# ittiam-systems/libxaac

Hardware: AMD Instinct MI355X
Metric: decoded audio frames/s (1024-spl IMDCT + complex QMF + HQ SBR + parametric stereo, HE-AACv2) (higher is better)
Workload: dtype int32

## Files before the change

libxaac_amd/csrc/sbr_ps_frame.h:

```cpp
#ifndef XAAC_SBR_PS_FRAME_H
#define XAAC_SBR_PS_FRAME_H

#include <stddef.h>

#include "sbr_ps.h"

#ifndef XP_T
#define XP_T(i)
#endif

#define XP_NO_PS_SCALE 0x7fffffff
#define XP_MAX_SEG (XAAC_PS_MAX_ENV + 2)

#if defined(__HIPCC__)
#define XP_UNROLL _Pragma("unroll")
#define XP_NOUNROLL _Pragma("nounroll")
#define XP_LAMBDA_INLINE __attribute__((always_inline))
#else
#define XP_UNROLL
#define XP_NOUNROLL
#define XP_LAMBDA_INLINE
#endif

struct XpFrameWork {
  union {
    int32_t hyb_u[3][2][44];
    int32_t gsum[8][56];
    int32_t peak[32][20];
    uint32_t dl[32][13];
  };
  int32_t hyb_l[32][20];
  union {
    int32_t binpw[32][20];
    int16_t ratio[32][20];
  };
  uint32_t ap_h[32][11];
  uint32_t seg_hd[XP_MAX_SEG][4][24];
};
template <bool B>
struct XpBool {
  static constexpr bool value = B;
};

FX_HD int xp_popc(uint32_t v) { return __builtin_popcount(v); }
FX_HD int xp_clz(uint32_t v) { return __builtin_clz(v); }
FX_HD uint32_t xp_pack16(int16_t lo, int16_t hi) { return (uint32_t)(uint16_t)lo | ((uint32_t)(uint16_t)hi << 16); }
FX_HD int16_t xp_lo16(uint32_t v) { return (int16_t)(v & 0xffffu); }
FX_HD int16_t xp_hi16(uint32_t v) { return (int16_t)(v >> 16); }

FX_HD int32_t xp_dot2(uint32_t a, uint32_t b) {
#if defined(__HIP_DEVICE_COMPILE__)
  int32_t r;
  asm("v_dot2_i32_i16 %0, %1, %2, 0" : "=v"(r) : "v"(a), "v"(b));
  return r;
#else
  return (int32_t)((uint32_t)((int32_t)xp_lo16(a) * xp_lo16(b)) + (uint32_t)((int32_t)xp_hi16(a) * xp_hi16(b)));
#endif
}
FX_HD int16_t xp_seg_coeff(uint32_t hd, int n) { return (int16_t)(xp_hi16(hd) + n * xp_lo16(hd)); }
FX_HD uint32_t xp_load_pair(const int16_t *p) {
#if defined(__HIP_DEVICE_COMPILE__)
  typedef uint32_t __attribute__((may_alias)) xp_u32_alias;
  return *reinterpret_cast<const xp_u32_alias *>(p);
#else
  return xp_pack16(p[0], p[1]);
#endif
}
struct XpPhase {
  uint32_t re_pair, im_pair;
};
FX_HD XpPhase xp_phase_pairs(int16_t re, int16_t im) {
  XpPhase p;
  p.re_pair = xp_pack16(re, (int16_t)-im);
  p.im_pair = xp_pack16(im, re);
  return p;
}
FX_HD uint32_t xp_q15_pair(int32_t a, int32_t b) {
  return (((uint32_t)a >> 15) & 0xffffu) | (((uint32_t)b << 1) & 0xffff0000u);
}
FX_HD uint32_t xp_hi_pair(int32_t a, int32_t b) {
#if defined(__HIP_DEVICE_COMPILE__)
  return __builtin_amdgcn_perm((uint32_t)b, (uint32_t)a, 0x07060302u);
#else
  return ((uint32_t)a >> 16) | ((uint32_t)b & 0xffff0000u);
#endif
}
FX_HD uint32_t xp_mult16_shl_pair(uint32_t p, int32_t f2) {
#if defined(__HIP_DEVICE_COMPILE__)
  return xp_hi_pair(__mul24(xp_lo16(p), f2), __mul24(xp_hi16(p), f2));
#else
  return xp_hi_pair((int32_t)((uint32_t)(int32_t)xp_lo16(p) * (uint32_t)f2), (int32_t)((uint32_t)(int32_t)xp_hi16(p) * (uint32_t)f2));
#endif
}
FX_HD int32_t xp_m16x16_shl_pre(int16_t a, int32_t b2) {
#if defined(__HIP_DEVICE_COMPILE__)
  return __mul24(a, b2);
#else
  return (int32_t)((uint32_t)(int32_t)a * (uint32_t)b2);
#endif
}
FX_HD uint32_t xp_add16_pair(uint32_t a, uint32_t b) {
#if defined(__HIP_DEVICE_COMPILE__)
  typedef short xp_short2 __attribute__((ext_vector_type(2)));
  return __builtin_bit_cast(uint32_t, (xp_short2)(__builtin_bit_cast(xp_short2, a) + __builtin_bit_cast(xp_short2, b)));
#else
  return ((a + b) & 0xffffu) | ((a & 0xffff0000u) + (b & 0xffff0000u));
#endif
}
FX_HD uint32_t xp_sub16_pair(uint32_t a, uint32_t b) {
#if defined(__HIP_DEVICE_COMPILE__)
  typedef short xp_short2 __attribute__((ext_vector_type(2)));
  return __builtin_bit_cast(uint32_t, (xp_short2)(__builtin_bit_cast(xp_short2, a) - __builtin_bit_cast(xp_short2, b)));
#else
  return ((a - b) & 0xffffu) | ((a & 0xffff0000u) - (b & 0xffff0000u));
#endif
}
FX_HD uint32_t xp_allpass_packed(uint32_t &d0, uint32_t new_pair, const XpPhase &ph, uint32_t &e0, uint32_t &e1, uint32_t &e2,
                                 const XpPhase &p0, const XpPhase &p1, const XpPhase &p2, int16_t decay0, int16_t decay1,
                                 int16_t decay2) {
  uint32_t in = xp_q15_pair(xp_dot2(d0, ph.re_pair), xp_dot2(d0, ph.im_pair));
  d0 = new_pair;
  uint32_t *e[3] = {&e0, &e1, &e2};
  const XpPhase *pp[3] = {&p0, &p1, &p2};
  const int32_t decay2x[3] = {2 * decay0, 2 * decay1, 2 * decay2};
  XP_UNROLL
  for (int m = 0; m < 3; m++) {
    const uint32_t s = *e[m];
    const uint32_t t = xp_sub16_pair(xp_q15_pair(xp_dot2(s, pp[m]->re_pair), xp_dot2(s, pp[m]->im_pair)),
                                     xp_mult16_shl_pair(in, decay2x[m]));
    *e[m] = xp_add16_pair(in, xp_mult16_shl_pair(t, decay2x[m]));
    in = t;
  }
  return in;
}

FX_HD int32_t xp_adj_word(int32_t v, int shift) {
  if (shift > 31) shift = 31;
  if (shift < -31) shift = -31;
  const int shl = shift > 0 ? shift : 0, shr = shift < 0 ? -shift : 0;
  return (int32_t)((uint32_t)v << shl) >> shr;
}

FX_HD int32_t xp_bin_power_hyb(const XpTables *T, int bin, const int32_t *re, const int32_t *im) {
  if (bin < 2) {
    const int a = bin == 0 ? 0 : 4, b = bin == 0 ? 5 : 1;
    int32_t pw = xp_power(re[a], im[a]);
    pw = fx_add_sat(pw, fx_mul32x16(re[b], (int16_t)(re[b] >> 16)));
    return fx_add_sat(pw, fx_mul32x16(im[b], (int16_t)(im[b] >> 16)));
  }
  const int sb = T->borders_group[bin + 2];
  return xp_power(re[sb], im[sb]);
}

template <int NS = 32, class PS>
FX_HD int xp_ps_frame(const XsCx &cx, const XpTables *T, PS *ps, const xaac_ps_frame *pf, XpFrameWork *w, int32_t *xl,
                      int32_t *xr, int lb_scale, int ov_lb_scale, int hb_scale, int st_syn, int lsb, int usb,
                      int ps_scale_done = XP_NO_PS_SCALE) {
  static_assert(NS == 32 || NS == 30, "frames of 32 or 30 QMF slots");
#if defined(__HIP_DEVICE_COMPILE__)
  int32_t p1v[3][2], p3re[32], p3im[32];
  {
    const int l1 = cx.lane & 31;
    XP_UNROLL
    for (int b = 0; b < 3; b++) {
      p1v[b][0] = xl[(l1 + 6) * 128 + b];
      p1v[b][1] = xl[(l1 + 6) * 128 + 64 + b];
    }
    XP_UNROLL
    for (int l = 0; l < 32; l++) {
      p3re[l] = NS == 32 || l < NS ? xl[l * 128 + cx.lane] : 0;
      p3im[l] = NS == 32 || l < NS ? xl[l * 128 + 64 + cx.lane] : 0;
    }
  }
#endif
  const int ps_scale = ps_scale_done != XP_NO_PS_SCALE ? ps_scale_done : xp_init_ps_scale(cx, ps, lb_scale, ov_lb_scale, hb_scale);
  const int ov_lb_shift = ps_scale - ov_lb_scale, lb_shift = ps_scale - lb_scale, hb_shift = ps_scale - hb_scale;
  const int common_shift = (st_syn - ps_scale) - 8;
  XP_T(1);

  XS_PAR(l, 0, NS) {
    const int shiftdelay = l < NS - 6 ? 0 : (int16_t)(lb_scale - ps_scale);
    for (int b = 0; b < 3; b++) {
      const int sha = l + 6 < NS ? (b < lsb ? lb_shift : (b < usb ? hb_shift : 0)) : 0;
      for (int c = 0; c < 2; c++) {
#if defined(__HIP_DEVICE_COMPILE__)
        int32_t v = xp_adj_word(p1v[b][c], sha);
#else
        int32_t v = xp_adj_word(xl[(l + 6) * 128 + 64 * c + b], sha);
#endif
        v = shiftdelay < 0 ? fx_shl(v, -shiftdelay) : fx_shr(v, shiftdelay);
        w->hyb_u[b][c][12 + l] = v;
      }
    }
  }
  XS_PAR(i, 0, 12)
    for (int b = 0; b < 3; b++) {
      w->hyb_u[b][0][i] = ps->hyb_buf[b][0][i];
      w->hyb_u[b][1][i] = ps->hyb_buf[b][1][i];
    }
  cx.sync();
  XS_PAR(l, 0, NS) {
    int32_t re[8], im[8];
    xp_filt_8ch(T, &w->hyb_u[0][0][l], &w->hyb_u[0][1][l], re, im);
    for (int k = 0; k < 6; k++) {
      w->hyb_l[l][k] = re[k];
      w->hyb_l[l][10 + k] = im[k];
    }
  }
  XS_PAR(i, 0, 64) {
    const int b = 1 + (i >> 5), l = i & 31;
    if (NS != 32 && l >= NS) continue;
    int32_t re[2], im[2];
    xp_filt_2ch(T, &w->hyb_u[b][0][l], &w->hyb_u[b][1][l], re, im);
    w->hyb_l[l][4 + 2 * b] = re[0];
    w->hyb_l[l][5 + 2 * b] = re[1];
    w->hyb_l[l][14 + 2 * b] = im[0];
    w->hyb_l[l][15 + 2 * b] = im[1];
  }
  XS_PAR(i, 0, 12)
    for (int b = 0; b < 3; b++) {
      ps->hyb_buf[b][0][i] = w->hyb_u[b][0][NS + i];
      ps->hyb_buf[b][1][i] = w->hyb_u[b][1][NS + i];
    }
  cx.sync();
  XP_T(2);

  XS_PAR(g, 0, XAAC_PS_GROUPS) {
    w->seg_hd[0][0][g] = xp_pack16(ps->delta_h11_h12[2 * g], ps->H11_H12[2 * g]);
    w->seg_hd[0][1][g] = xp_pack16(ps->delta_h11_h12[2 * g + 1], ps->H11_H12[2 * g + 1]);
    w->seg_hd[0][2][g] = xp_pack16(ps->delta_h21_h22[2 * g], ps->H21_H22[2 * g]);
    w->seg_hd[0][3][g] = xp_pack16(ps->delta_h21_h22[2 * g + 1], ps->H21_H22[2 * g + 1]);
  }
  const int usb_prev = cx.uni(ps->usb);
  uint32_t seg_mask = 0;
  int clear_slot = NS;
  {
    int env = 0, nseg = 1;
    int next = cx.uni(pf->border_position[0]);
    for (int l = 0; l < NS; l++) {
      if (l == next) {
        if (env == 0) clear_slot = l;
        cx.sync();
        xp_rot_env_coeffs(cx, T, ps, pf, env);
        XS_PAR(g, 0, XAAC_PS_GROUPS) {
          w->seg_hd[nseg][0][g] = xp_pack16(ps->delta_h11_h12[2 * g], ps->H11_H12[2 * g]);
          w->seg_hd[nseg][1][g] = xp_pack16(ps->delta_h11_h12[2 * g + 1], ps->H11_H12[2 * g + 1]);
          w->seg_hd[nseg][2][g] = xp_pack16(ps->delta_h21_h22[2 * g], ps->H21_H22[2 * g]);
          w->seg_hd[nseg][3][g] = xp_pack16(ps->delta_h21_h22[2 * g + 1], ps->H21_H22[2 * g + 1]);
        }
        seg_mask |= 1u << l;
        nseg++;
        env++;
        next = env <= XAAC_PS_MAX_ENV ? cx.uni(pf->border_position[env]) : 64;
      }
    }
  }
  cx.sync();
  XP_T(3);

  {
    XP_UNROLL
    for (int c = 0; c < 4; c++) {
      XS_PAR(sb, 0, 64) {
        int32_t rre[8], rim[8];
        XP_UNROLL
        for (int ls = 0; ls < 8; ls++) {
#if defined(__HIP_DEVICE_COMPILE__)
          rre[ls] = p3re[8 * c + ls];
          rim[ls] = p3im[8 * c + ls];
#else
          rre[ls] = xl[(8 * c + ls) * 128 + sb];
          rim[ls] = xl[(8 * c + ls) * 128 + 64 + sb];
#endif
        }
        const int gsh = sb < 11 ? 0 : (sb < 18 ? 1 : (sb < 23 ? 2 : (sb < 35 ? 3 : 4)));
        const bool own_bin = sb >= 3 && sb < 9;
        int32_t *dst = sb < 3 ? &w->gsum[0][55] : (own_bin ? &w->binpw[8 * c][sb + 5] : &w->gsum[0][sb - 9]);
        const int dstride = own_bin ? 20 : 56;
        XP_UNROLL
        for (int ls = 0; ls < 8; ls++) {
          const int l = 8 * c + ls;
          const int usb_l = l >= clear_slot ? usb : usb_prev;
          const int sh = sb < lsb ? (l < 6 ? ov_lb_shift : lb_shift) : (sb < usb ? hb_shift : 0);
          const int32_t re = xp_adj_word(rre[ls], sh), im = xp_adj_word(rim[ls], sh);
          const int32_t pw = xp_power(re, im);
          dst[ls * dstride] = own_bin ? pw : (sb < usb_l ? (pw >> gsh) : 0);
        }
      }
      cx.sync();
      XS_PAR(i, 0, 48) {
        const int ls = i / 6, g = i % 6;
        const int b0 = T->borders_group[16 + g], b1 = T->borders_group[17 + g];
        int32_t acc = 0;
#if defined(__HIP_DEVICE_COMPILE__) && !defined(XP_OLD_GSUM)
        for (int sb = b0; sb < b1; sb += 8) {
          int32_t t[8];
          XP_UNROLL
          for (int j = 0; j < 8; j++) t[j] = w->gsum[ls][(sb + j < b1 ? sb + j : b1 - 1) - 9];
          XP_UNROLL
          for (int j = 0; j < 8; j++) acc = fx_add_sat(acc, sb + j < b1 ? t[j] : 0);
        }
#else
        for (int sb = b0; sb < b1; sb++) acc = fx_add_sat(acc, w->gsum[ls][sb - 9]);
#endif
        w->binpw[8 * c + ls][14 + g] = acc;
      }
      cx.sync();
    }
  }
  XS_PAR(i, 0, 8 * NS) {
    const int l = i >> 3, bin = i & 7;
    w->binpw[l][bin] = xp_bin_power_hyb(T, bin, &w->hyb_l[l][0], &w->hyb_l[l][10]);
  }
  cx.sync();
  XP_T(4);

  XS_PAR(bin, 0, 20) {
    int32_t pd = ps->peak_decay_diff[bin], pdp = ps->peak_decay_diff_prev[bin], nrg = ps->energy_prev[bin];
    int32_t pin[NS];
    XP_UNROLL
    for (int l = 0; l < NS; l++) pin[l] = w->binpw[l][bin];
    XP_UNROLL
    for (int l = 0; l < NS; l++) {
      int32_t pw = fx_shl(pin[l], 1);
      if (pw < 0) pw = 0;
      pd = fx_mul32x16_shl(pd, 0x620a);
      if (pw > pd) pd = pw;
      pdp = fx_add_sat(fx_mul32x16_shl(pdp, 0x6000), fx_sub_sat(pd, pw) >> 2);
      nrg = fx_add_sat(fx_mul32x16_shl(nrg, 0x6000), pw >> 2);
      w->binpw[l][bin] = nrg;
      w->peak[l][bin] = fx_add_sat(pdp, pdp >> 1);
    }
    ps->peak_decay_diff[bin] = pd;
    ps->peak_decay_diff_prev[bin] = pdp;
    ps->energy_prev[bin] = nrg;
  }
  cx.sync();
  for (int i0 = 0; i0 < 20 * NS; i0 += 64) {
    int16_t q = 0;
    XS_PAR(i, i0, (20 * NS) % 64 == 0 || i0 + 64 < 20 * NS ? i0 + 64 : 20 * NS) {
      const int32_t pk = (&w->peak[0][0])[i], nrg = (&w->binpw[0][0])[i];
      q = pk <= nrg ? (int16_t)0x7fff : (int16_t)xp_divide16_pos(nrg, pk);
#if !defined(__HIP_DEVICE_COMPILE__)
      (&w->ratio[0][0])[i] = q;
#endif
    }
#if defined(__HIP_DEVICE_COMPILE__)
    cx.sync();
    (&w->ratio[0][0])[i0 + cx.lane] = q;
    cx.sync();
#endif
  }
  cx.sync();
  XP_T(5);

  {
    const int idx0 = cx.uni(ps->idx), idx_long0 = cx.uni(ps->idx_long);
    const int is0 = cx.uni(ps->idx_ser[0]), is1 = cx.uni(ps->idx_ser[1]), is2 = cx.uni(ps->idx_ser[2]);
    const int clear_lo = (usb > usb_prev && usb_prev) ? usb_prev : 64;
    const int clear_hi = usb < 23 ? usb : 23;
    const int p14_0 = idx_long0 % 14;
    const int cs_right = common_shift < 0 ? (-common_shift > 31 ? 31 : -common_shift) : 0;
    uint32_t events = seg_mask | (1u << 6) | (1u << 14);
    if (clear_slot < NS) events |= 1u << clear_slot;
    if (clear_slot + 14 < NS) events |= 1u << (clear_slot + 14);
    XS_PAR(sb, 0, 64) {
      const int qmf_chain = sb >= 3 && sb < 23, hyb_chain = sb >= 32 && sb < 42, chain = qmf_chain || hyb_chain;
      const int csb = qmf_chain ? sb : (hyb_chain ? sb - 32 : 3);
      const int di = 9 + 3 * (csb - 3);
      const int16_t *ph = hyb_chain ? &T->frac_delay_phase_fac_qmf_sub_re_im[2 * csb] : &T->frac_delay_phase_fac_qmf_re_im[2 * csb];
      const int16_t *pser = hyb_chain ? &T->frac_delay_phase_fac_qmf_sub_ser_re_im[2 * csb] : &T->frac_delay_phase_fac_qmf_ser_re_im[2 * csb];
      const int pstep = hyb_chain ? 32 : 64;
      const XpPhase phase = xp_phase_pairs(ph[0], ph[1]);
      const XpPhase ps0 = xp_phase_pairs(pser[0], pser[1]), ps1 = xp_phase_pairs(pser[pstep], pser[pstep + 1]),
                    ps2 = xp_phase_pairs(pser[2 * pstep], pser[2 * pstep + 1]);
      const int16_t dec0 = hyb_chain ? T->rev_link_decay_ser[0] : T->decay_scale_factor[qmf_chain ? di : 9];
      const int16_t dec1 = hyb_chain ? T->rev_link_decay_ser[1] : T->decay_scale_factor[qmf_chain ? di + 1 : 10];
      const int16_t dec2 = hyb_chain ? T->rev_link_decay_ser[2] : T->decay_scale_factor[qmf_chain ? di + 2 : 11];
      uint32_t d0[2] = {0, 0}, r0[3] = {0, 0, 0}, r1[4] = {0, 0, 0, 0}, r2[5] = {0, 0, 0, 0, 0};
      if (chain) {
        XP_UNROLL
        for (int j = 0; j < 2; j++) {
          const int16_t *q = hyb_chain ? &ps->sub[(idx0 + j) % 2][2 * csb] : &ps->ap[(idx0 + j) % 2][2 * csb];
          d0[j] = xp_pack16(q[0], q[1]);
        }
        XP_UNROLL
        for (int j = 0; j < 3; j++) {
          const int16_t *q = hyb_chain ? &ps->sub_ser[(is0 + j) % 3][0][2 * csb] : &ps->ser[(is0 + j) % 3][0][2 * csb];
          r0[j] = xp_pack16(q[0], q[1]);
        }
        XP_UNROLL
        for (int j = 0; j < 4; j++) {
          const int16_t *q = hyb_chain ? &ps->sub_ser[(is1 + j) % 4][1][2 * csb] : &ps->ser[(is1 + j) % 4][1][2 * csb];
          r1[j] = xp_pack16(q[0], q[1]);
        }
        XP_UNROLL
        for (int j = 0; j < 5; j++) {
          const int16_t *q = hyb_chain ? &ps->sub_ser[(is2 + j) % 5][2][2 * csb] : &ps->ser[(is2 + j) % 5][2][2 * csb];
          r2[j] = xp_pack16(q[0], q[1]);
        }
      }
      const int g = T->band_to_group[sb];
      const int bin_sb = sb < 23 ? T->delay_to_bin[sb] : (sb < 35 ? 18 : 19);
      uint32_t h11, h12, h21, h22, d11, d12, d21, d22;
      const auto seg_load = [&](int s) {
        const uint32_t a = w->seg_hd[s][0][g], b = w->seg_hd[s][1][g], c = w->seg_hd[s][2][g], d = w->seg_hd[s][3][g];
        h11 = a & 0xffff0000u, h12 = b & 0xffff0000u, h21 = c & 0xffff0000u, h22 = d & 0xffff0000u;
        d11 = a << 16, d12 = b << 16, d21 = c << 16, d22 = d << 16;
      };
      seg_load(0);
      uint32_t prev = sb >= 35 ? xp_pack16(ps->sd[2 * (sb - 35)], ps->sd[2 * (sb - 35) + 1]) : 0u;
      const int is_ap = sb < 23, is_d14 = sb >= 23 && sb < 35;
      int shl_ov, shr_ov, shl_lb, shr_lb;
      {
        const int s_ov = sb < lsb ? ov_lb_shift : (sb < usb ? hb_shift : 0), s_lb = sb < lsb ? lb_shift : (sb < usb ? hb_shift : 0);
        const int c_ov = s_ov > 31 ? 31 : (s_ov < -31 ? -31 : s_ov), c_lb = s_lb > 31 ? 31 : (s_lb < -31 ? -31 : s_lb);
        shl_ov = c_ov > 0 ? c_ov : 0, shr_ov = c_ov < 0 ? -c_ov : 0;
        shl_lb = c_lb > 0 ? c_lb : 0, shr_lb = c_lb < 0 ? -c_lb : 0;
      }
      int shl = shl_ov, shr = shr_ov;
      bool active = sb < usb_prev, fed14 = false;
      const int ldj = is_d14 ? 2 * (sb - 23) : 0, dlj = is_d14 ? sb - 23 : 12, apj = hyb_chain ? csb : 10;
      int ld_at = 24 * p14_0;
      const int16_t *const ld_lane = &ps->ld[0][ldj];
      static_assert(sizeof(ps->ld[0]) == 24 * sizeof(int16_t), "rows of the 14-slot ring: 24 int16, whole words");
      static_assert(offsetof(PS, ld) % 4 == 0 && alignof(PS) % 4 == 0, "the 14-slot ring starts on a word of a word-aligned state");
      int16_t tr_nx = w->ratio[0][bin_sb];
      int32_t hre_nx = w->hyb_l[0][csb], him_nx = w->hyb_l[0][10 + csb];
      uint32_t ld_nx = xp_load_pair(ld_lane + ld_at);
      int32_t nre[4], nim[4];
      XP_UNROLL
      for (int j = 0; j < 4; j++) {
        nre[j] = xl[j * 128 + sb];
        nim[j] = xl[j * 128 + 64 + sb];
      }
      const auto walk = [&](auto cs_positive) XP_LAMBDA_INLINE {
        XP_NOUNROLL
        for (int l0 = 0; l0 < NS; l0 += 4) {
          int32_t cre[4], cim[4];
          XP_UNROLL
          for (int j = 0; j < 4; j++) {
            cre[j] = nre[j];
            cim[j] = nim[j];
          }
          if (l0 + 4 < NS) {
            XP_UNROLL
            for (int j = 0; j < 4; j++) {
              nre[j] = xl[(l0 + 4 + j) * 128 + sb];
              nim[j] = xl[(l0 + 4 + j) * 128 + 64 + sb];
            }
          }
          const uint32_t events4 = events >> l0;
          XP_UNROLL
          for (int j = 0; j < 4; j++) {
            const int l = l0 + j;
            if (NS % 4 != 0 && l >= NS) break;
            const int16_t tr = tr_nx;
            const int32_t hre = hre_nx, him = him_nx;
            const uint32_t ld_cur = ld_nx;
            {
              const int ln = l + 1 < NS ? l + 1 : NS - 1;
              ld_at = ld_at + 24 == 14 * 24 ? 0 : ld_at + 24;
              tr_nx = w->ratio[ln][bin_sb];
              hre_nx = w->hyb_l[ln][csb];
              him_nx = w->hyb_l[ln][10 + csb];
              ld_nx = xp_load_pair(ld_lane + ld_at);
            }
            if ((events4 >> j) & 1u) {
#if defined(__HIP_DEVICE_COMPILE__)
              asm volatile("");
#endif
              shl = l < 6 ? shl_ov : shl_lb;
              shr = l < 6 ? shr_ov : shr_lb;
              active = sb < (l >= clear_slot ? usb : usb_prev);
              fed14 = l >= 14 && sb < (l - 14 >= clear_slot ? usb : usb_prev);
              if (l == clear_slot) {
                const int c = qmf_chain && sb >= clear_lo && sb < clear_hi;
                XP_UNROLL
                for (int m = 0; m < 3; m++) r0[m] = c ? 0u : r0[m];
                XP_UNROLL
                for (int m = 0; m < 4; m++) r1[m] = c ? 0u : r1[m];
                XP_UNROLL
                for (int m = 0; m < 5; m++) r2[m] = c ? 0u : r2[m];
              }
              if ((seg_mask >> l) & 1u)
                seg_load(xp_popc(seg_mask & (0xffffffffu >> (31 - l))));
            }
            const int32_t re0 = (int32_t)((uint32_t)cre[j] << shl) >> shr, im0 = (int32_t)((uint32_t)cim[j] << shl) >> shr;
            const int16_t q_re = fx_round16(re0), q_im = fx_round16(im0);
            const uint32_t q = xp_pack16(q_re, q_im);
            const uint32_t in_pair = hyb_chain ? xp_pack16(fx_round16(hre), fx_round16(him)) : q;
            uint32_t dv = d0[0], e0 = r0[0], e1 = r1[0], e2 = r2[0];
            const uint32_t o_chain = xp_allpass_packed(dv, in_pair, phase, e0, e1, e2, ps0, ps1, ps2, dec0, dec1, dec2);
            d0[0] = d0[1];
            d0[1] = dv;
            r0[0] = r0[1]; r0[1] = r0[2];
            r0[2] = e0;
            r1[0] = r1[1]; r1[1] = r1[2]; r1[2] = r1[3];
            r1[3] = e1;
            r2[0] = r2[1]; r2[1] = r2[2]; r2[2] = r2[3]; r2[3] = r2[4];
            r2[4] = e2;
            w->ap_h[l][apj] = o_chain;
            h11 += d11;
            h12 += d12;
            h21 += d21;
            h22 += d22;
            const uint32_t o14_new = w->dl[l >= 14 ? l - 14 : 0][dlj];
            const uint32_t o14 = fed14 ? o14_new : ld_cur;
            const uint32_t o = is_ap ? o_chain : (is_d14 ? o14 : prev);
            w->dl[l][dlj] = q;
            prev = active ? q : prev;
            int32_t re = re0, im = im0;
            int32_t r_re = xp_m16x16_shl_pre(xp_lo16(o), 2 * tr), r_im = xp_m16x16_shl_pre(xp_hi16(o), 2 * tr);
            xp_rotate_w(&re, &r_re, h11, h12, h21, h22);
            xp_rotate_w(&im, &r_im, h11, h12, h21, h22);
            re = active ? re : re0;
            im = active ? im : im0;
            r_re = active ? r_re : 0;
            r_im = active ? r_im : 0;
            if (decltype(cs_positive)::value) {
              re = fx_shl_sat(re, common_shift);
              im = fx_shl_sat(im, common_shift);
            } else {
              re = re >> cs_right;
              im = im >> cs_right;
            }
            if (sb >= 3) {
              xl[l * 128 + sb] = re;
              xl[l * 128 + 64 + sb] = im;
              xr[l * 128 + sb] = r_re;
              xr[l * 128 + 64 + sb] = r_im;
            }
          }
        }
      };
      if (common_shift > 0)
        walk(XpBool<true>());
      else
        walk(XpBool<false>());
      if (chain) {
        XP_UNROLL
        for (int j = 0; j < 2; j++) {
          int16_t *q = hyb_chain ? &ps->sub[(idx0 + j) % 2][2 * csb] : &ps->ap[(idx0 + j) % 2][2 * csb];
          q[0] = xp_lo16(d0[j]);
          q[1] = xp_hi16(d0[j]);
        }
        XP_UNROLL
        for (int j = 0; j < 3; j++) {
          int16_t *q = hyb_chain ? &ps->sub_ser[(is0 + NS + j) % 3][0][2 * csb] : &ps->ser[(is0 + NS + j) % 3][0][2 * csb];
          q[0] = xp_lo16(r0[j]);
          q[1] = xp_hi16(r0[j]);
        }
        XP_UNROLL
        for (int j = 0; j < 4; j++) {
          int16_t *q = hyb_chain ? &ps->sub_ser[(is1 + NS + j) % 4][1][2 * csb] : &ps->ser[(is1 + NS + j) % 4][1][2 * csb];
          q[0] = xp_lo16(r1[j]);
          q[1] = xp_hi16(r1[j]);
        }
        XP_UNROLL
        for (int j = 0; j < 5; j++) {
          int16_t *q = hyb_chain ? &ps->sub_ser[(is2 + NS + j) % 5][2][2 * csb] : &ps->ser[(is2 + NS + j) % 5][2][2 * csb];
          q[0] = xp_lo16(r2[j]);
          q[1] = xp_hi16(r2[j]);
        }
      }
      if (sb >= 35) {
        ps->sd[2 * (sb - 35)] = xp_lo16(prev);
        ps->sd[2 * (sb - 35) + 1] = xp_hi16(prev);
      }
      if (is_d14) {
        for (int l = (clear_slot == 0 || usb == usb_prev) ? NS - 14 : 0; l < NS; l++) {
          const int pos = (idx_long0 + l) % 14;
          if (sb < (l >= clear_slot ? usb : usb_prev)) {
            ps->ld[pos][ldj] = xp_lo16(w->dl[l][dlj]);
            ps->ld[pos][ldj + 1] = xp_hi16(w->dl[l][dlj]);
          }
        }
      }
    }
    cx.sync();
    XS_ONE {
      ps->idx = (int16_t)idx0;
      ps->idx_ser[0] = (int16_t)((is0 + NS) % 3);
      ps->idx_ser[1] = (int16_t)((is1 + NS) % 4);
      ps->idx_ser[2] = (int16_t)((is2 + NS) % 5);
      ps->idx_long = (int16_t)((idx_long0 + NS) % 14);
      if (clear_slot < NS) ps->usb = (int16_t)usb;
    }
  }
  cx.sync();
  XP_T(6);

  XS_PAR(i, 0, 6 * NS) {
    const int l = i / 6, b = (i % 6) >> 1, c = i & 1;
    const int p = b == 0 ? 0 : 4 + 2 * b, n = b == 0 ? 6 : 2;
    const uint32_t below = seg_mask & (0xffffffffu >> (31 - l));
    const int s = xp_popc(below), nn = l - (below ? 31 - xp_clz(below) : 0) + 1;
    int32_t acc_l = 0, acc_r = 0;
    for (int k = 0; k < n; k++) {
      const int sb = p + k;
      const int16_t h11 = xp_seg_coeff(w->seg_hd[s][0][sb], nn), h12 = xp_seg_coeff(w->seg_hd[s][1][sb], nn);
      const int16_t h21 = xp_seg_coeff(w->seg_hd[s][2][sb], nn), h22 = xp_seg_coeff(w->seg_hd[s][3][sb], nn);
      const int16_t tr = w->ratio[l][T->hybrid_to_bin[sb]];
      const uint32_t o = w->ap_h[l][sb];
      int32_t lv = w->hyb_l[l][10 * c + sb];
      int32_t rv = xp_m16x16_shl(c ? xp_hi16(o) : xp_lo16(o), tr);
      xp_rotate(&lv, &rv, h11, h12, h21, h22);
      acc_l = k == 0 ? lv : fx_add_sat(acc_l, lv);
      acc_r = k == 0 ? rv : fx_add_sat(acc_r, rv);
    }
    if (common_shift < 0)
      acc_l = fx_shr(acc_l, -common_shift > 31 ? 31 : -common_shift);
    else if (common_shift > 0)
      acc_l = fx_shl_sat(acc_l, common_shift);
    xl[l * 128 + 64 * c + b] = acc_l;
    xr[l * 128 + 64 * c + b] = acc_r;
  }
  {
    const int s = xp_popc(seg_mask), n = NS - (seg_mask ? 31 - xp_clz(seg_mask) : 0);
    XS_PAR(g, 0, XAAC_PS_GROUPS) {
      ps->H11_H12[2 * g] = xp_seg_coeff(w->seg_hd[s][0][g], n);
      ps->H11_H12[2 * g + 1] = xp_seg_coeff(w->seg_hd[s][1][g], n);
      ps->H21_H22[2 * g] = xp_seg_coeff(w->seg_hd[s][2][g], n);
      ps->H21_H22[2 * g + 1] = xp_seg_coeff(w->seg_hd[s][3][g], n);
    }
  }
  cx.sync();
  XP_T(7);
  return ps_scale;
}

#endif
```

Baseline: 17.54 million.

## Replace shared-memory group power sums with DPP wavefront prefix scan

Group power sums are now built with an in-register DPP prefix scan across the 64 subband lanes. Only each group's last-lane prefix is written to a small scan table, and the group sums come from differences of adjacent prefixes. This removes the per-chunk gsum buffer, the 48-thread reduction pass and two block syncs per chunk, leaving one sync after all chunks. Separately, hybrid synthesis now gives one thread per slot and channel, which accumulates all three bins in one unrolled loop. The trade-offs are wrapping unsigned arithmetic with a final clamp instead of per-add saturation, and a reliance on GFX9 row_bcast DPP controls and a 64-lane wavefront.

```diff
diff --git a/libxaac_amd/csrc/sbr_ps_frame.h b/libxaac_amd/csrc/sbr_ps_frame.h
--- a/libxaac_amd/csrc/sbr_ps_frame.h
+++ b/libxaac_amd/csrc/sbr_ps_frame.h
@@ -25,7 +25,7 @@
 struct XpFrameWork {
   union {
     int32_t hyb_u[3][2][44];
-    int32_t gsum[8][56];
+    uint32_t gscan[32][8];
     int32_t peak[32][20];
     uint32_t dl[32][13];
   };
@@ -150,6 +150,41 @@
   }
   const int sb = T->borders_group[bin + 2];
   return xp_power(re[sb], im[sb]);
+}
+
+FX_HD uint32_t xp_gsum_addend(int32_t pw, int group_shift, bool counts) { return counts ? (uint32_t)(pw >> group_shift) : 0u; }
+FX_HD uint32_t xp_gsum_scan(const XsCx &cx, uint32_t a, uint32_t &run) {
+#if defined(__HIP_DEVICE_COMPILE__)
+  int32_t r = (int32_t)a;
+#define XP_DPP_ADD(ctrl, rows) r += __builtin_amdgcn_update_dpp(0, r, ctrl, rows, 0xf, false);
+  XP_DPP_ADD(0x111, 0xf)
+  XP_DPP_ADD(0x112, 0xf)
+  XP_DPP_ADD(0x114, 0xf)
+  XP_DPP_ADD(0x118, 0xf)
+  XP_DPP_ADD(0x142, 0xa)
+  XP_DPP_ADD(0x143, 0xc)
+#undef XP_DPP_ADD
+  (void)cx;
+  (void)run;
+  return (uint32_t)r;
+#else
+  (void)cx;
+  run += a;
+  return run;
+#endif
+}
+FX_HD int32_t xp_gsum_sum(uint32_t s_last, uint32_t s_before) {
+  const uint32_t d = s_last - s_before;
+  return (int32_t)(d < 0x7fffffffu ? d : 0x7fffffffu);
+}
+FX_HD bool xp_gsum_fits(const XpTables *T) {
+  if (T->borders_group[16] != 9) return false;
+  for (int g = 0; g < 6; g++) {
+    const int b0 = T->borders_group[16 + g], b1 = T->borders_group[17 + g], shift = T->group_shift[g];
+    if (b1 <= b0 || b1 > 64 || shift < 0 || shift > 31) return false;
+    if ((uint64_t)(b1 - b0) * (uint64_t)(0x7fffffff >> shift) >= ((uint64_t)1 << 32)) return false;
+  }
+  return true;
 }
 
 template <int NS = 32, class PS>
@@ -261,6 +296,7 @@
   {
     XP_UNROLL
     for (int c = 0; c < 4; c++) {
+      uint32_t run[8] = {0, 0, 0, 0, 0, 0, 0, 0};
       XS_PAR(sb, 0, 64) {
         int32_t rre[8], rim[8];
         XP_UNROLL
@@ -275,8 +311,11 @@
         }
         const int gsh = sb < 11 ? 0 : (sb < 18 ? 1 : (sb < 23 ? 2 : (sb < 35 ? 3 : 4)));
         const bool own_bin = sb >= 3 && sb < 9;
-        int32_t *dst = sb < 3 ? &w->gsum[0][55] : (own_bin ? &w->binpw[8 * c][sb + 5] : &w->gsum[0][sb - 9]);
-        const int dstride = own_bin ? 20 : 56;
+        int gcol = 6;
+        XP_UNROLL
+        for (int g = 0; g < 6; g++) gcol = sb == T->borders_group[17 + g] - 1 ? g : gcol;
+        int32_t *dst = own_bin ? &w->binpw[8 * c][sb + 5] : reinterpret_cast<int32_t *>(&w->gscan[8 * c][gcol]);
+        const int dstride = own_bin ? 20 : 8;
         XP_UNROLL
         for (int ls = 0; ls < 8; ls++) {
           const int l = 8 * c + ls;
@@ -284,29 +323,18 @@
           const int sh = sb < lsb ? (l < 6 ? ov_lb_shift : lb_shift) : (sb < usb ? hb_shift : 0);
           const int32_t re = xp_adj_word(rre[ls], sh), im = xp_adj_word(rim[ls], sh);
           const int32_t pw = xp_power(re, im);
-          dst[ls * dstride] = own_bin ? pw : (sb < usb_l ? (pw >> gsh) : 0);
-        }
-      }
-      cx.sync();
-      XS_PAR(i, 0, 48) {
-        const int ls = i / 6, g = i % 6;
-        const int b0 = T->borders_group[16 + g], b1 = T->borders_group[17 + g];
-        int32_t acc = 0;
-#if defined(__HIP_DEVICE_COMPILE__) && !defined(XP_OLD_GSUM)
-        for (int sb = b0; sb < b1; sb += 8) {
-          int32_t t[8];
-          XP_UNROLL
-          for (int j = 0; j < 8; j++) t[j] = w->gsum[ls][(sb + j < b1 ? sb + j : b1 - 1) - 9];
-          XP_UNROLL
-          for (int j = 0; j < 8; j++) acc = fx_add_sat(acc, sb + j < b1 ? t[j] : 0);
-        }
-#else
-        for (int sb = b0; sb < b1; sb++) acc = fx_add_sat(acc, w->gsum[ls][sb - 9]);
-#endif
-        w->binpw[8 * c + ls][14 + g] = acc;
-      }
-      cx.sync();
-    }
+          const uint32_t s = xp_gsum_scan(cx, xp_gsum_addend(pw, gsh, sb >= 9 && sb < usb_l), run[ls]);
+          dst[ls * dstride] = own_bin ? pw : (int32_t)s;
+        }
+      }
+    }
+  }
+  cx.sync();
+  XS_PAR(i, 0, 6 * NS) {
+    const int l = i / 6, g = i % 6;
+    const uint32_t prev = w->gscan[l][g > 0 ? g - 1 : 0];
+    const uint32_t before = g > 0 ? prev : 0u;
+    w->binpw[l][14 + g] = xp_gsum_sum(w->gscan[l][g], before);
   }
   XS_PAR(i, 0, 8 * NS) {
     const int l = i >> 3, bin = i & 7;
@@ -591,14 +619,15 @@
   cx.sync();
   XP_T(6);
 
-  XS_PAR(i, 0, 6 * NS) {
-    const int l = i / 6, b = (i % 6) >> 1, c = i & 1;
-    const int p = b == 0 ? 0 : 4 + 2 * b, n = b == 0 ? 6 : 2;
+  XS_PAR(i, 0, 2 * NS) {
+    const int l = i >> 1, c = i & 1;
     const uint32_t below = seg_mask & (0xffffffffu >> (31 - l));
     const int s = xp_popc(below), nn = l - (below ? 31 - xp_clz(below) : 0) + 1;
-    int32_t acc_l = 0, acc_r = 0;
-    for (int k = 0; k < n; k++) {
-      const int sb = p + k;
+    int32_t acc_l[3] = {0, 0, 0}, acc_r[3] = {0, 0, 0};
+    XP_UNROLL
+    for (int sb = 0; sb < 10; sb++) {
+      const int b = sb < 6 ? 0 : (sb < 8 ? 1 : 2);
+      const bool first = sb == 0 || sb == 6 || sb == 8;
       const int16_t h11 = xp_seg_coeff(w->seg_hd[s][0][sb], nn), h12 = xp_seg_coeff(w->seg_hd[s][1][sb], nn);
       const int16_t h21 = xp_seg_coeff(w->seg_hd[s][2][sb], nn), h22 = xp_seg_coeff(w->seg_hd[s][3][sb], nn);
       const int16_t tr = w->ratio[l][T->hybrid_to_bin[sb]];
@@ -606,15 +635,19 @@
       int32_t lv = w->hyb_l[l][10 * c + sb];
       int32_t rv = xp_m16x16_shl(c ? xp_hi16(o) : xp_lo16(o), tr);
       xp_rotate(&lv, &rv, h11, h12, h21, h22);
-      acc_l = k == 0 ? lv : fx_add_sat(acc_l, lv);
-      acc_r = k == 0 ? rv : fx_add_sat(acc_r, rv);
-    }
-    if (common_shift < 0)
-      acc_l = fx_shr(acc_l, -common_shift > 31 ? 31 : -common_shift);
-    else if (common_shift > 0)
-      acc_l = fx_shl_sat(acc_l, common_shift);
-    xl[l * 128 + 64 * c + b] = acc_l;
-    xr[l * 128 + 64 * c + b] = acc_r;
+      acc_l[b] = first ? lv : fx_add_sat(acc_l[b], lv);
+      acc_r[b] = first ? rv : fx_add_sat(acc_r[b], rv);
+    }
+    XP_UNROLL
+    for (int b = 0; b < 3; b++) {
+      int32_t v = acc_l[b];
+      if (common_shift < 0)
+        v = fx_shr(v, -common_shift > 31 ? 31 : -common_shift);
+      else if (common_shift > 0)
+        v = fx_shl_sat(v, common_shift);
+      xl[l * 128 + 64 * c + b] = v;
+      xr[l * 128 + 64 * c + b] = acc_r[b];
+    }
   }
   {
     const int s = xp_popc(seg_mask), n = NS - (seg_mask ? 31 - xp_clz(seg_mask) : 0);
```

After: 17.95 million (median of 6 runs). 2.3% higher.
